# lonelycorn/mvSLAM

Measured on AMD Instinct MI355X. Metric: image-pairs/sec (2k kp, 50k RANSAC hyp), higher is better.
Workload: dtype f64; 1 GPU; 512 independent synthetic 640x480 pairs per GPU, 2000 keypoints (256-bit descriptors), 50000 8-point hypotheses per pair, full match+RANSAC+decompose+triangulate; pairs_per_gpu=512, keypoints=2000, hypotheses=50000, parallelism=pairs sharded, dp1, streams=2

## Files before the change

mvslam_amd/csrc/capi.hip:

```cpp
#include <dlfcn.h>
#include <hip/hip_runtime.h>

#include <algorithm>
#include <cmath>
#include <cstdio>
#include <cstdlib>
#include <cstring>
#include <functional>
#include <memory>
#include <string>
#include <type_traits>
#include <vector>

#include "kernels.hpp"

using namespace mvs;

struct HipFree {
    void operator()(void *p) const { (void)hipFree(p); }
};
using DevPtr = std::unique_ptr<void, HipFree>;
using DevBlocks = std::vector<DevPtr>;
struct DevWorkspace {
    DevPtr p;
// ... 208 lines not shown
static mvs_status ws_grow(mvs_ctx *ctx, DevWorkspace &w, size_t bytes, size_t floor = 0)
{
    if (w.bytes >= bytes)
        return MVS_OK;
    HIP_TRY(ctx, sync_stream(ctx));
    w.p.reset();
    w.bytes = 0;
    void *p = nullptr;
    HIP_TRY(ctx, hipMalloc(&p, std::max(bytes, floor)));
    w.p.reset(p);
    w.bytes = std::max(bytes, floor);
    return MVS_OK;
}

static void drop_orb_graph(mvs_ctx *ctx)
{
    if (ctx->orb_graph)
        (void)hipGraphExecDestroy(ctx->orb_graph);
    ctx->orb_graph = nullptr;
    ctx->orb_graph_valid = false;
}

struct Carve {
    size_t align, end = 0;
    size_t up(size_t x) const { return (x + align - 1) & ~(align - 1); }
    size_t take(size_t bytes)
    {
        const size_t o = up(end);
        end = o + bytes;
        return o;
    }
    size_t total() const { return up(end); }
};

static mvs_status ensure_groups(mvs_batch *b, int num_hypotheses)
{
    const int G = (num_hypotheses + kHypPerBlock - 1) / kHypPerBlock;
    if (G <= b->d.max_groups)
        return MVS_OK;
    HIP_TRY(b->ctx, sync_stream(b->ctx));
    const size_t P = (size_t)b->d.n_pairs, Hp = (size_t)G * kHypPerBlock;
    if (P * Hp >= (size_t(1) << 32))
        return MVS_ERR_CAPACITY;
    BatchDev &d = b->d;
    DevGroup g(b->ctx, b->blocks);
    g.add(d.wgbest, P * G);
    g.add(d.hyp_F, P * kHypRec * Hp);
    g.add(d.hyp_r32, P * kHypRec32 * Hp);
    g.add(d.hyp_okf, P * Hp);
    g.add(d.hyp_cnt, P * Hp);
    g.add(d.xlist, P * Hp);
    g.add(d.clist, 2 * P * Hp);
    if (!d.bound) g.add(d.bound, P);
    if (!d.box) g.add(d.box, P * 8);
    if (!d.mode) g.add(d.mode, P);
    if (!d.dense_n1) g.add(d.dense_n1, P);
    if (!d.ccount) g.add(d.ccount, P);
    if (!d.pcount) g.add(d.pcount, P);
    if (!d.cpos) g.add(d.cpos, P * kSortBins);
    if (!d.m0list) g.add(d.m0list, 2 * (P + 1));
    if (!d.xcount) g.add(d.xcount, 4);
    const mvs_status st = g.commit();
    if (st != MVS_OK)
        return st;
    d.clist2 = d.clist + P * Hp;
    d.max_groups = G;
    return MVS_OK;
}

static mvs_status alloc_refine(mvs_ctx *ctx, DevBlocks &owner, RefineDev &d, int problems, int stride, int frames,
                               const double *K)
{
    const size_t T = problems, S = stride;
    RefineDev r{};
    r.n_problems = problems;
    r.stride = stride;
    r.n_frames = frames;
    r.K = K;
    DevGroup g(ctx, owner);
    for (int f = 0; f < frames; ++f) {
        g.add(r.obs[f], T * S * 2);
        g.add(r.oinfo[f], T * S * 3);
    }
    g.add(r.pts0, T * S * 3);
    g.add(r.pinfo, T * S * 6);
    g.add(r.pts, T * S * 3);
    g.add(r.pts_tmp, T * S * 3);
    if (frames == 2)
        g.add(r.point_cov, T * S * 9);
    g.add(r.pose0, T * 12);
    g.add(r.m, T);
    g.add(r.out, T);
    const mvs_status st = g.commit();
    if (st == MVS_OK)
        d = r;
    return st;
}

#ifdef MVS_DEBUG_HOOKS
template <typename Launch>
static int probe_io(mvs_ctx *ctx, const void *const *in, const size_t *in_bytes, int n_in, void *const *outp, const size_t *out_bytes,
                    int n_out, Launch launch)
{
    HIP_TRY(ctx, hipSetDevice(ctx->device));
    unsigned char *d[8] = {};
    DevBlocks tmp;
    DevGroup g(ctx, tmp);
// ... 657 lines not shown
    return MVS_OK;
}

mvs_status mvs_batch_upload(mvs_batch *b, int first, int count, const uint8_t *base_desc, const float *base_kp,
                            const int32_t *n_base, const uint8_t *pair_desc, const float *pair_kp,
                            const int32_t *n_pair, const double *K, const int64_t *global_index)
{
    return batch_upload_impl(b, first, count, base_desc, base_kp, n_base, pair_desc, pair_kp, n_pair, K, global_index, true);
}

mvs_status mvs_batch_upload_async(mvs_batch *b, int first, int count, const uint8_t *base_desc, const float *base_kp,
                                  const int32_t *n_base, const uint8_t *pair_desc, const float *pair_kp,
                                  const int32_t *n_pair, const double *K, const int64_t *global_index)
{
    return batch_upload_impl(b, first, count, base_desc, base_kp, n_base, pair_desc, pair_kp, n_pair, K, global_index, false);
}

mvs_status mvs_host_alloc(size_t bytes, void **out)
{
    if (!out || bytes == 0)
        return MVS_ERR_INVALID_ARG;
    *out = nullptr;
    return hipHostMalloc(out, bytes, hipHostMallocPortable) == hipSuccess ? MVS_OK : MVS_ERR_HIP;
}

void mvs_host_free(void *p)
{
    if (p)
        (void)hipHostFree(p);
}

static mvs_status check_params(const mvs_params *p)
{
    if (!p || p->num_hypotheses < 1 || (p->sampler != MVS_SAMPLER_IDENTITY && p->sampler != MVS_SAMPLER_PHILOX))
        return MVS_ERR_INVALID_ARG;
    return MVS_OK;
}

static BatchDev batch_view(const BatchDev &b, int first, int count, int half)
{
    BatchDev v = b;
    const size_t f = (size_t)first, N = (size_t)b.max_kp, Hp = (size_t)b.max_groups * kHypPerBlock;
    v.n_pairs = count;
    v.desc1 += f * N * b.desc_words; v.desc2 += f * N * b.desc_words;
    v.kp1 += f * N * 2; v.kp2 += f * N * 2;
    v.oct1 += f * N; v.oct2 += f * N;
    v.n1 += f; v.n2 += f;
    v.Kinv += f * 9; v.K += f * 9; v.gidx += f;
    v.knn_train += f * N; v.knn_dist += f * N;
    v.M += f; v.matches += f * N; v.pts += f * N * 4;
    v.wgbest += f * b.max_groups;
    v.hyp_F += f * Hp * kHypRec; v.hyp_r32 += f * Hp * kHypRec32;
    v.hyp_okf += f * Hp; v.hyp_cnt += f * Hp;
    v.bound += f; v.box += f * 8; v.mode += f;
    v.clist += f * Hp; v.clist2 += f * Hp; v.cpos += f * kSortBins;
    v.ccount += f; v.pcount += f; v.dense_n1 += f;
    v.m0list += (size_t)half * ((size_t)b.n_pairs + 1);
    v.xlist += f * Hp;
    v.xcount += 2 * half;
    v.cand_pts += f * 4 * N * 3; v.fin += f; v.inl += f * N; v.okf += f * 4 * N;
    v.results += f; v.mask += f * N; v.points += f * N * 3; v.point_idx += f * N;
    return v;
}

constexpr int kHalvesMinPairs = 64;

static void enqueue_stages(const BatchDev &d, const RunParams &rp, int n_active, bool stats, hipStream_t s, hipEvent_t *ev,
                           LaunchTimer *lt, bool with_match = true)
{
    if (ev) (void)hipEventRecord(ev[0], s);
    if (with_match)
        launch_match_topk(d, rp, n_active, s, lt);
    if (ev) (void)hipEventRecord(ev[1], s);
    if (with_match)
        launch_match_compact(d, rp, n_active, s, lt);
    if (ev) (void)hipEventRecord(ev[2], s);
    launch_ransac(d, rp, n_active, stats, s, lt);
    if (ev) (void)hipEventRecord(ev[3], s);
    launch_finalize(d, rp, n_active, kFinalizeFull, s, lt);
    if (ev) (void)hipEventRecord(ev[4], s);
}

static mvs_status enqueue_pipeline(mvs_batch *b, const RunParams &rp, int n_active, bool stats, hipEvent_t *ev,
                                   LaunchTimer *lt = nullptr, bool with_match = true)
{
    mvs_ctx *ctx = b->ctx;
    hipStream_t s = ctx->stream;
    const bool halves = n_active >= kHalvesMinPairs && !stats && !ev && !lt && !b->d.hyp_count && ctx->half_batches;
    if (!halves) {
        enqueue_stages(b->d, rp, n_active, stats, s, ev, lt, with_match);
    } else {
        const int na = (n_active + 1) / 2;
        HIP_TRY(ctx, hipEventRecord(ctx->ev_fork, s));
        HIP_TRY(ctx, hipStreamWaitEvent(ctx->side, ctx->ev_fork, 0));
        enqueue_stages(batch_view(b->d, 0, na, 0), rp, na, false, s, nullptr, nullptr, with_match);
        const hipError_t e_first = hipGetLastError();
        enqueue_stages(batch_view(b->d, na, n_active - na, 1), rp, n_active - na, false, ctx->side, nullptr, nullptr, with_match);
        const hipError_t e_second = hipGetLastError();
        hipError_t e_join = hipEventRecord(ctx->ev_join, ctx->side);
        if (e_join == hipSuccess)
            e_join = hipStreamWaitEvent(s, ctx->ev_join, 0);
        if (e_join != hipSuccess)
            (void)hipStreamSynchronize(ctx->side);
        HIP_TRY(ctx, e_first);
        HIP_TRY(ctx, e_second);
        HIP_TRY(ctx, e_join);
    }
// ... 2196 lines not shown
```

mvslam_amd/csrc/device_math.hpp:

```cpp
#pragma once
#include <hip/hip_runtime.h>
#include <stdint.h>

#define MVS_DEV __device__ __forceinline__

namespace mvs {

constexpr double kEps = 2.220446049250313e-16;
constexpr double kTol = kEps * 1000.0;
constexpr double kJacobiEps = kEps * 10.0;
constexpr double kMinVal = 2.2250738585072014e-308;
constexpr double kSqrt2 = 1.4142135623730951;

MVS_DEV double dfma(double a, double b, double c) { return __builtin_fma(a, b, c); }
MVS_DEV double dsqrt(double a) { return __builtin_sqrt(a); }
MVS_DEV double dabs(double a) { return __builtin_fabs(a); }

MVS_DEV void rotate_inplace(double &x, double &y, double c, double s)
{
    double t0, t1;
    asm("v_mul_f64 %0, %4, %3\n\t"
        "v_mul_f64 %1, %4, %2\n\t"
        "v_fma_f64 %3, %5, %3, -%1\n\t"
        "v_fma_f64 %2, %5, %2, %0"
// ... 317 lines not shown
        double sd = W[i];
        for (int ii = 0; ii < 100 && sd <= kMinVal; ++ii) {
            const double val0 = 1.0 / 3.0;
#pragma unroll
            for (int k = 0; k < 3; ++k)
                At[i][k] = (cvrng_next(rng) & 256u) != 0 ? val0 : -val0;
#pragma unroll
            for (int it = 0; it < 2; ++it) {
#pragma unroll
                for (int j = 0; j < 3; ++j) {
                    if (j < i) {
                        sd = 0.0;
#pragma unroll
                        for (int k = 0; k < 3; ++k)
                            sd += At[i][k] * At[j][k];
                        double asum = 0.0;
#pragma unroll
                        for (int k = 0; k < 3; ++k) {
                            const double t = At[i][k] - sd * At[j][k];
                            At[i][k] = t;
                            asum += dabs(t);
                        }
                        asum = asum > kJacobiEps * 100.0 ? 1.0 / asum : 0.0;
#pragma unroll
                        for (int k = 0; k < 3; ++k)
                            At[i][k] *= asum;
                    }
                }
            }
            sd = 0.0;
#pragma unroll
            for (int k = 0; k < 3; ++k)
                sd += At[i][k] * At[i][k];
            sd = dsqrt(sd);
        }
        const double s = sd > kMinVal ? 1.0 / sd : 0.0;
#pragma unroll
        for (int k = 0; k < 3; ++k)
            At[i][k] *= s;
    }
#pragma unroll
    for (int i = 0; i < 3; ++i)
#pragma unroll
        for (int j = 0; j < 3; ++j)
            U[i][j] = At[j][i];
}
MVS_DEV void svd3_full(const double (&A)[3][3], double (&w)[3], double (&U)[3][3], double (&Vt)[3][3], unsigned &rot,
                       unsigned &pairs)
{
    bool bad3 = false;
    svd3_full<false, false, false>(A, w, U, Vt, rot, pairs, bad3);
}

MVS_DEV void philox4x32_10(uint32_t c0, uint32_t c1, uint32_t c2, uint32_t c3, uint32_t k0, uint32_t k1,
                           uint32_t (&out)[4])
{
#pragma unroll
    for (int r = 0; r < 10; ++r) {
        const uint64_t p0 = (uint64_t)0xD2511F53u * c0, p1 = (uint64_t)0xCD9E8D57u * c2;
        const uint32_t hi0 = (uint32_t)(p0 >> 32), lo0 = (uint32_t)p0;
        const uint32_t hi1 = (uint32_t)(p1 >> 32), lo1 = (uint32_t)p1;
        const uint32_t n0 = hi1 ^ c1 ^ k0, n2 = hi0 ^ c3 ^ k1;
        c0 = n0; c1 = lo1; c2 = n2; c3 = lo0;
        k0 += 0x9E3779B9u;
        k1 += 0xBB67AE85u;
    }
    out[0] = c0; out[1] = c1; out[2] = c2; out[3] = c3;
}

MVS_DEV void sample8(uint64_t seed, uint32_t hyp, int M, int sampler, int (&idx)[8])
{
    if (sampler == 0) {
#pragma unroll
        for (int k = 0; k < 8; ++k)
            idx[k] = k;
        return;
    }
    uint32_t w[8];
    {
        uint32_t o[4];
        philox4x32_10(hyp, 0u, 0u, 0u, (uint32_t)seed, (uint32_t)(seed >> 32), o);
        w[0] = o[0]; w[1] = o[1]; w[2] = o[2]; w[3] = o[3];
        philox4x32_10(hyp, 1u, 0u, 0u, (uint32_t)seed, (uint32_t)(seed >> 32), o);
        w[4] = o[0]; w[5] = o[1]; w[6] = o[2]; w[7] = o[3];
    }
    int sorted[8];
#pragma unroll
    for (int k = 0; k < 8; ++k)
        sorted[k] = 0x7fffffff;
#pragma unroll
    for (int k = 0; k < 8; ++k) {
        uint32_t r = __umulhi(w[k], (uint32_t)(M - k));
#pragma unroll
        for (int t = 0; t < 8; ++t)
            if (t < k && r >= (uint32_t)sorted[t])
                ++r;
        idx[k] = (int)r;
        int carry = (int)r;
#pragma unroll
        for (int t = 0; t < 8; ++t) {
            if (t <= k) {
                const int cur = sorted[t];
                const bool sw = carry < cur;
                sorted[t] = sw ? carry : cur;
                carry = sw ? cur : carry;
            }
        }
    }
}

MVS_DEV bool normalise8(const double (&px)[8], const double (&py)[8], double (&nx)[8], double (&ny)[8], double &scale,
                        double &mx, double &my)
{
    mx = 0.0;
    my = 0.0;
#pragma unroll
    for (int i = 0; i < 8; ++i) {
        mx += px[i];
        my += py[i];
    }
    mx *= 0.125;
    my *= 0.125;
    double sc = 0.0;
#pragma unroll
    for (int i = 0; i < 8; ++i) {
        const double dx = px[i] - mx, dy = py[i] - my;
        nx[i] = dx;
        ny[i] = dy;
        sc += dsqrt(dx * dx + dy * dy);
    }
    sc *= 0.125;
    const bool ok = sc > kEps;
    sc = kSqrt2 / sc;
#pragma unroll
    for (int i = 0; i < 8; ++i) {
        nx[i] *= sc;
        ny[i] *= sc;
    }
    scale = sc;
    return ok;
}

struct EightNorm {
    double s1, s2, m1x, m1y, m2x, m2y;
};

MVS_DEV bool eight_point_front(const double (&x1)[8], const double (&y1)[8], const double (&x2)[8], const double (&y2)[8],
                               double (&At)[9][9], EightNorm &nm)
{
    double a1[8], b1[8], a2[8], b2[8];
    bool ok = normalise8(x1, y1, a1, b1, nm.s1, nm.m1x, nm.m1y);
    ok = normalise8(x2, y2, a2, b2, nm.s2, nm.m2x, nm.m2y) && ok;
    double A[8][9];
#pragma unroll
    for (int i = 0; i < 8; ++i) {
        A[i][0] = a2[i] * a1[i]; A[i][1] = a2[i] * b1[i]; A[i][2] = a2[i];
        A[i][3] = b2[i] * a1[i]; A[i][4] = b2[i] * b1[i]; A[i][5] = b2[i];
        A[i][6] = a1[i];         A[i][7] = b1[i];         A[i][8] = 1.0;
    }
#pragma unroll
    for (int i = 0; i < 9; ++i) {
#pragma unroll
// ... 109 lines not shown
```

mvslam_amd/csrc/kernels.hip:

```cpp
#include <algorithm>
#include "kernels.hpp"

#include "device_math.hpp"
#include "prescreen.hpp"

namespace mvs {

constexpr uint32_t kKeyNone = 0xffffffffu;
__device__ __forceinline__ uint32_t bcnt_acc(uint32_t x, uint32_t acc)
{
    uint32_t r;
    asm("v_bcnt_u32_b32 %0, %1, %2" : "=v"(r) : "v"(x), "v"(acc));
    return r;
}
__device__ __forceinline__ void key_insert(uint32_t &k0, uint32_t &k1, uint32_t k)
{
    uint32_t m;
    asm("v_med3_u32 %0, %1, %2, %3" : "=v"(m) : "v"(k0), "v"(k1), "v"(k));
    k1 = m;
    k0 = min(k0, k);
}

constexpr int kTopkWaves = 16;
constexpr int kTopkTileBytes = 65536;
// ... 538 lines not shown
    for (int k = 0; k < 9; ++k)
        Fo[k] = F[k];
    Fo[9] = pair_max_error_sq(b, rp, pair);
    b.hyp_okf[(size_t)pair * Hp + h] = ok ? kPsExact : kPsInvalid;
    if (h == 0)
        b.bound[pair] = 0;
}


__global__ __launch_bounds__(256) void mode0_list_kernel(BatchDev b, int n_active)
{
    __shared__ int s_cnt[4];
    __shared__ int s_total;
    const int tid = threadIdx.x, lane = tid & 63, w = tid >> 6;
    if (tid == 0)
        s_total = 0;
    __syncthreads();
    for (int p0 = 0; p0 < n_active; p0 += 256) {
        const int pair = p0 + tid;
        const bool take = pair < n_active && b.M[pair] >= 8 && b.mode[pair] == 0;
        const unsigned long long m = __ballot(take);
        if (lane == 0)
            s_cnt[w] = __popcll(m);
        __syncthreads();
        int base = s_total;
        for (int k = 0; k < w; ++k)
            base += s_cnt[k];
        if (take)
            b.m0list[1 + base + __popcll(m & ((1ull << lane) - 1ull))] = pair;
        __syncthreads();
        if (tid == 0)
            s_total += s_cnt[0] + s_cnt[1] + s_cnt[2] + s_cnt[3];
        __syncthreads();
    }
    if (tid == 0)
        b.m0list[0] = s_total;
}

__global__ __launch_bounds__(256, 1) void ransac_solve_list_kernel(BatchDev b, RunParams rp, int blocks_per_pair)
{
    const int n_items = b.m0list[0] * blocks_per_pair;
    for (int item = blockIdx.x; item < n_items; item += gridDim.x) {
        const int pair = b.m0list[1 + item / blocks_per_pair];
        solve_record(b, rp, pair, b.M[pair], (uint32_t)(item % blocks_per_pair) * 64u + threadIdx.x);
    }
}

constexpr int kCntSlots = 4;
typedef __attribute__((address_space(4))) double CDouble;


__device__ __forceinline__ PairBox load_box(const BatchDev &b, int pair)
{
    const double *q = b.box + (size_t)pair * 8;
    PairBox bx;
    bx.x1lo = q[0]; bx.x1hi = q[1]; bx.y1lo = q[2]; bx.y1hi = q[3];
    bx.x2lo = q[4]; bx.x2hi = q[5]; bx.y2lo = q[6]; bx.y2hi = q[7];
    return bx;
}

__device__ __forceinline__ int prescreen_sample(uint64_t seed, uint32_t hyp, int M, int sampler, const double *P, double *park,
                                                const PairBox &bx, double thr, double (&F)[9], double &band, double &e32,
                                                bool &bad3)
{
    int idx[8];
    sample8(seed, hyp, M, sampler, idx);
    return prescreen_hypothesis(P, idx, park, bx, thr, F, band, e32, bad3);
}

__global__ __launch_bounds__(256) void pair_prepare_kernel(BatchDev b, RunParams rp, int force_mode)
{
    __shared__ double s_red[4][8];
    __shared__ double s_park[kPsParked * 64];
    const int pair = blockIdx.x, tid = threadIdx.x, lane = tid & 63, w = tid >> 6;
    const int M = min(b.M[pair], b.max_kp);
    if (pair == 0 && tid < 2)
        b.xcount[tid] = 0u;
    if (tid == 0) {
        b.bound[pair] = 0;
        b.ccount[pair] = 0;
        b.pcount[pair] = 0;
    }
    if (M < 8) {
        if (tid == 0)
            b.mode[pair] = 0;
        return;
    }
    const double4 *P4 = reinterpret_cast<const double4 *>(b.pts + (size_t)pair * b.max_kp * 4);
    const double big = 0x1p1000;
    double lo[4] = {big, big, big, big}, hi[4] = {-big, -big, -big, -big};
    for (int i = tid; i < M; i += 256) {
        const double4 p = P4[i];
        const double v[4] = {p.x, p.y, p.z, p.w};
#pragma unroll
        for (int k = 0; k < 4; ++k) {
            lo[k] = fmin(lo[k], v[k]);
            hi[k] = fmax(hi[k], v[k]);
        }
    }
#pragma unroll
    for (int k = 0; k < 4; ++k) {
#pragma unroll
        for (int o = 32; o > 0; o >>= 1) {
            lo[k] = fmin(lo[k], __shfl_xor(lo[k], o));
            hi[k] = fmax(hi[k], __shfl_xor(hi[k], o));
        }
    }
    if (lane == 0) {
#pragma unroll
        for (int k = 0; k < 4; ++k) {
            s_red[w][2 * k] = lo[k];
            s_red[w][2 * k + 1] = hi[k];
        }
    }
    __syncthreads();
    PairBox bx;
    {
        double q[8];
#pragma unroll
        for (int k = 0; k < 8; ++k) {
            const double a0 = s_red[0][k], a1 = s_red[1][k], a2 = s_red[2][k], a3 = s_red[3][k];
            q[k] = (k & 1) ? fmax(fmax(a0, a1), fmax(a2, a3)) : fmin(fmin(a0, a1), fmin(a2, a3));
        }
        bx.x1lo = q[0]; bx.x1hi = q[1]; bx.y1lo = q[2]; bx.y1hi = q[3];
        bx.x2lo = q[4]; bx.x2hi = q[5]; bx.y2lo = q[6]; bx.y2hi = q[7];
        if (tid < 8)
            b.box[(size_t)pair * 8 + tid] = q[tid];
    }
    if (w == 0) {
        const int H = rp.num_hypotheses;
        const uint64_t seed = rp.seed + (uint64_t)b.gidx[pair];
        const double thr = pair_max_error_sq(b, rp, pair);
        const uint32_t hh = (uint32_t)min(lane, H - 1);
        double F[9], band, e32;
        bool bad3 = false;
        int flag = prescreen_sample(seed, hh, M, rp.sampler, reinterpret_cast<const double *>(P4), s_park + lane, bx, thr, F, band, e32,
                                    bad3);
        if (bad3 && flag == kPsApprox)
            flag = kPsNeedExact;
        const bool live = lane < H;
        const int n_ok = __popcll(__ballot(live && flag != kPsInvalid));
        const int n_s64 = __popcll(__ballot(live && flag == kPsApprox && band <= kPsProbeFrac * thr));
        const int n_s32 = __popcll(__ballot(live && flag == kPsApprox && band + e32 <= kPsProbeFrac * thr &&
                                            band + 65.0 * e32 <= kPsProbeMfmaFrac * thr));
        const int mode = n_ok == 0 ? 0 : 3 * n_s32 >= n_ok ? 1 : 3 * n_s64 >= n_ok ? 2 : 0;
        if (lane == 0)
            b.mode[pair] = force_mode >= 0 ? force_mode : mode;
    }
}

__global__ __launch_bounds__(64) __attribute__((amdgpu_waves_per_eu(3, 3))) void ransac_prescreen_kernel(BatchDev b, RunParams rp)
{
    __shared__ double s_park[kPsParked * 64];
    const int pair = blockIdx.y, lane = threadIdx.x;
    const int M = b.M[pair];
    if (M < 8 || b.mode[pair] == 0)
        return;
    const int H = rp.num_hypotheses;
    const uint32_t h = blockIdx.x * 64 + lane;
    const bool live = h < (uint32_t)H;
    const uint32_t hh = live ? h : (uint32_t)(H - 1);
    const uint64_t seed = rp.seed + (uint64_t)b.gidx[pair];
    const double *P = b.pts + (size_t)pair * b.max_kp * 4;
    const PairBox bx = load_box(b, pair);
    const double thr = pair_max_error_sq(b, rp, pair);
    double F[9], band, e32;
    bool bad3 = false;
    int flag = prescreen_sample(seed, hh, M, rp.sampler, P, s_park + lane, bx, thr, F, band, e32, bad3);
    const int mode = b.mode[pair];
    const double btot = mode == 1 ? band + e32 : band;
    if (flag == kPsApprox && (bad3 || !(btot <= kPsBandFrac * thr)))
        flag = kPsNeedExact;
    if (!live)
        flag = kPsInvalid;
    const size_t Hp = (size_t)b.max_groups * kHypPerBlock;
    const size_t rec = (size_t)pair * Hp + h;
    double *Fo = b.hyp_F + rec * kHypRec;
    if (mode == 1) {
        float *fo = b.hyp_r32 + rec * kHypRec32;
        float q[12];
// ... 1112 lines not shown
                        F[k] = f[k];
                    c = 0;
#pragma unroll 4
                    for (int i = 0; i < M; ++i) {
                        const double4 p = L4[i];
                        c += epipolar_residual(F, p.x, p.y, p.z, p.w) < thr ? 1 : 0;
                    }
                }
                s_cnt[q] = c;
            }
        } else if (b.mode[pair] != 0) {
            for (int q = w; q < n_list; q += kSelThreads / 64) {
                if (okb[s_list[q]] == kPsInvalid) {
                    if (lane == 0)
                        s_cnt[q] = -1;
                    continue;
                }
                const double *f = Fp + (size_t)s_list[q] * kHypRec;
                double F[9];
#pragma unroll
                for (int k = 0; k < 9; ++k)
                    F[k] = f[k];
                int c = 0;
                for (int i = lane; i < M; i += 64) {
                    const double4 p = P4[i];
                    c += epipolar_residual(F, p.x, p.y, p.z, p.w) < thr ? 1 : 0;
                }
#pragma unroll
                for (int o = 32; o > 0; o >>= 1)
                    c += __shfl_xor(c, o);
                if (lane == 0)
                    s_cnt[q] = c;
            }
        } else {
            for (int q = tid; q < n_list; q += kSelThreads)
                s_cnt[q] = cntp[s_list[q]];
        }
        __syncthreads();
        {
            int cm = -1;
            for (int q = tid; q < n_list; q += kSelThreads)
                cm = max(cm, s_cnt[q]);
#pragma unroll
            for (int o = 32; o > 0; o >>= 1)
                cm = max(cm, __shfl_xor(cm, o));
            if (lane == 0)
                s_tot[w] = cm;
            __syncthreads();
            const int target = max(max(max(s_tot[0], s_tot[1]), max(s_tot[2], s_tot[3])), s_best.cnt);
            __syncthreads();
            int n_ties = 0;
            for (int q0 = 0; q0 < n_list; q0 += kSelThreads) {
                const int q = q0 + tid;
                const bool tie = q < n_list && s_cnt[q] == target;
                const uint32_t hq = q < n_list ? s_list[q] : 0u;
                const unsigned long long bal = __ballot(tie);
                if (lane == 0)
                    s_tot[w] = __popcll(bal);
                __syncthreads();
                int off = n_ties, tot = 0;
#pragma unroll
                for (int k = 0; k < 4; ++k) {
                    const int v = s_tot[k];
                    off += (k < w) ? v : 0;
                    tot += v;
                }
                if (tie)
                    s_list[off + __popcll(bal & ((1ull << lane) - 1ull))] = hq;
                n_ties += tot;
                __syncthreads();
            }
            n_list = n_ties;
        }
        if (n_list == 0)
            continue;
        if (n_list <= kSelSerial) {
            staged = false;
            for (int q = 0; q < n_list; ++q) {
                const uint32_t h = s_list[q];
                if (tid < 9)
                    s_F[tid] = Fp[(size_t)h * kHypRec + tid];
                __syncthreads();
                double F[9];
#pragma unroll
                for (int k = 0; k < 9; ++k)
                    F[k] = s_F[k];
                int n_in = 0;
                for (int start = 0; start < M; start += kSelThreads) {
                    const int i = start + tid;
                    double r = 0.0;
                    bool in = false;
                    if (i < M) {
                        const double4 p = P4[i];
                        r = epipolar_residual(F, p.x, p.y, p.z, p.w);
                        in = r < thr;
                    }
                    const unsigned long long bal = __ballot(in);
                    if (lane == 0)
                        s_tot[w] = __popcll(bal);
                    __syncthreads();
                    int off = n_in, tot = 0;
#pragma unroll
                    for (int k = 0; k < 4; ++k) {
                        const int v = s_tot[k];
                        off += (k < w) ? v : 0;
                        tot += v;
                    }
// ... 1010 lines not shown
```

mvslam_amd/csrc/kernels.hpp:

```cpp
#pragma once
#include <hip/hip_runtime.h>
#include <stdint.h>

#include "../../include/mvslam_hip.h"

namespace mvs {

constexpr int kMaxKp = 4096;
constexpr int kSortBins = kMaxKp + 1;
constexpr int kHypPerBlock = 256;
constexpr int kMaxDescWords = 16;
constexpr int kHypRec = 10;
constexpr int kHypRec32 = 12;

struct WgBest {
    int32_t count;
    uint32_t hyp;
    double residual;
    double F[9];
};
static_assert(sizeof(WgBest) == 88, "WgBest layout");

struct FinModel {
    double R[2][9];
    double Rr[2][9];
    double T[3];
    int32_t n_inl;
    int32_t ncand;
    int32_t proceed;
    int32_t npre;
    int32_t pre_cnt[4];
    int32_t best_c;
    int32_t pad[3];
};

struct BatchDev {
    int n_pairs;
    int max_kp;
    int desc_words;
    int max_groups;
    int cu_count;

    const uint32_t *desc1;
    const uint32_t *desc2;
    const float *kp1;
    const float *kp2;
    const uint8_t *oct1;
    const uint8_t *oct2;
    const int32_t *n1;
    const int32_t *n2;
    const double *Kinv;
    const double *K;
    const int64_t *gidx;

    int32_t *knn_train;
    int32_t *knn_dist;
    int32_t *M;
    mvs_match *matches;
    double *pts;
    WgBest *wgbest;
// ... 342 lines not shown
```

mvslam_amd/csrc/prescreen.hpp:

```cpp
#pragma once
#include "device_math.hpp"

namespace mvs {

struct PairBox {
    double x1lo, x1hi, y1lo, y1hi, x2lo, x2hi, y2lo, y2hi;
};

constexpr double kPsU = 0x1p-53;
constexpr double kPsTauC = 2.0e-12;
constexpr double kPsEtaQ = 4.0e-12;
constexpr double kPsSvd3 = 2.0e-11;
constexpr double kPsTrip = 1.0e-12;
constexpr double kPsBandFrac = 4.0;
constexpr double kPsProbeFrac = 0.125;
constexpr double kPsProbeMfmaFrac = 1.25;
constexpr int kPsInvalid = 0, kPsApprox = 1, kPsNeedExact = 2, kPsExact = 3;

MVS_DEV double recip_guarded(double x) { return div_fast(1.0, x); }

MVS_DEV double sqrt_bound(double x)
{
    const double y = __builtin_amdgcn_rsq(x);
    double g = x * y;
    const double h = y * 0.5;
    const double r = dfma(-h, g, 0.5);
    g = dfma(g, r, g);
    const double d = dfma(-g, g, x);
    return dfma(d, h, g);
}
MVS_DEV double sqrt_bound0(double x)
{
    const double g = sqrt_bound(x);
    return x < 0x1p-700 ? 0.0 : g;
}
MVS_DEV double rcp_bound(double x)
{
    double r = __builtin_amdgcn_rcp(x);
    double e = dfma(-x, r, 1.0);
    r = dfma(r, e, r);
    e = dfma(-x, r, 1.0);
    return dfma(r, e, r);
}

MVS_DEV bool sample_norm(const double (&px)[8], const double (&py)[8], double &scale, double &mx, double &my, bool &tiny)
{
    mx = 0.0;
    my = 0.0;
#pragma unroll
    for (int i = 0; i < 8; ++i) {
        mx += px[i];
        my += py[i];
    }
    mx *= 0.125;
    my *= 0.125;
    double sc = 0.0;
#pragma unroll
    for (int i = 0; i < 8; ++i) {
        const double dx = px[i] - mx, dy = py[i] - my;
        const double q = dx * dx + dy * dy;
        tiny = tiny | ((q != 0.0) & !sqrt_fast_ok(q));
        sc += sqrt_fast(q);
    }
    sc *= 0.125;
    const bool ok = sc > kEps;
    scale = kSqrt2 / sc;
    return ok;
}

MVS_DEV void prescreen_rank2(const double (&g)[9], double (&X)[9], double &e_out, double &sige_out, double &extra_out,
                             double &s2lb_out, bool &ok_out)
{
    const double c00 = dfma(g[6], g[6], dfma(g[3], g[3], g[0] * g[0]));
    const double c01 = dfma(g[6], g[7], dfma(g[3], g[4], g[0] * g[1]));
    const double c02 = dfma(g[6], g[8], dfma(g[3], g[5], g[0] * g[2]));
    const double c11 = dfma(g[7], g[7], dfma(g[4], g[4], g[1] * g[1]));
    const double c12 = dfma(g[7], g[8], dfma(g[4], g[5], g[1] * g[2]));
    const double c22 = dfma(g[8], g[8], dfma(g[5], g[5], g[2] * g[2]));
    const double k2 = (c00 + c11) + c22;
    const double k1 = dfma(c00, c11, -(c01 * c01)) + dfma(c00, c22, -(c02 * c02)) + dfma(c11, c22, -(c12 * c12));
    const double dg = dfma(g[0], dfma(g[4], g[8], -(g[5] * g[7])),
                           dfma(-g[1], dfma(g[3], g[8], -(g[5] * g[6])), g[2] * dfma(g[3], g[7], -(g[4] * g[6]))));
    const double k0 = dg * dg;
    const double m2k2 = -2.0 * k2;
    double lam = 0.0;
#pragma unroll
    for (int it = 0; it < 8; ++it) {
        const double f = dfma(dfma(lam - k2, lam, k1), lam, -k0);
        const double fp = dfma(dfma(3.0, lam, m2k2), lam, k1);
        double r = __builtin_amdgcn_rcp(fp);
        r = r * dfma(-fp, r, 2.0);
        lam = dfma(-f, r, lam);
    }
    const double m00 = c00 - lam, m11 = c11 - lam, m22 = c22 - lam;
    const double ax = dfma(c01, c12, -(c02 * m11)), ay = dfma(c02, c01, -(m00 * c12)), az = dfma(m00, m11, -(c01 * c01));
    const double bx = dfma(c01, m22, -(c02 * c12)), by = dfma(c02, c02, -(m00 * m22)), bz = dfma(m00, c12, -(c01 * c02));
    const double cx = dfma(m11, m22, -(c12 * c12)), cy = dfma(c12, c02, -(c01 * m22)), cz = dfma(c01, c12, -(m11 * c02));
    const double na = dfma(az, az, dfma(ay, ay, ax * ax));
    const double nb = dfma(bz, bz, dfma(by, by, bx * bx));
    const double nc = dfma(cz, cz, dfma(cy, cy, cx * cx));
    const bool ub = nb > na;
    double vx = ub ? bx : ax, vy = ub ? by : ay, vz = ub ? bz : az, nv = ub ? nb : na;
    const bool uc = nc > nv;
    vx = uc ? cx : vx; vy = uc ? cy : vy; vz = uc ? cz : vz; nv = uc ? nc : nv;
    bool ok = nv >= 0x1p-190;
    double h;
    (void)sqrt_fast_nz_h(nv, h);
    h += h;
    vx *= h; vy *= h; vz *= h;
    const double w0 = dfma(g[2], vz, dfma(g[1], vy, g[0] * vx));
    const double w1 = dfma(g[5], vz, dfma(g[4], vy, g[3] * vx));
    const double w2 = dfma(g[8], vz, dfma(g[7], vy, g[6] * vx));
    X[0] = dfma(-w0, vx, g[0]); X[1] = dfma(-w0, vy, g[1]); X[2] = dfma(-w0, vz, g[2]);
    X[3] = dfma(-w1, vx, g[3]); X[4] = dfma(-w1, vy, g[4]); X[5] = dfma(-w1, vz, g[5]);
    X[6] = dfma(-w2, vx, g[6]); X[7] = dfma(-w2, vy, g[7]); X[8] = dfma(-w2, vz, g[8]);
    const double sg2 = dfma(w2, w2, dfma(w1, w1, w0 * w0));
    const double sig = dsqrt(sg2);
    const double rs = div_fast(1.0, fmax(sig, 0x1p-190));
    const double u0 = w0 * rs, u1 = w1 * rs, u2 = w2 * rs;
    const double e0 = dfma(g[6], u2, dfma(g[3], u1, dfma(g[0], u0, -(sig * vx))));
// ... 1 lines not shown
    const double e2 = dfma(g[8], u2, dfma(g[5], u1, dfma(g[2], u0, -(sig * vz))));
    const double eps2 = sqrt_bound0(dfma(e2, e2, dfma(e1, e1, e0 * e0))) * (1.0 + 1e-14);
    const bool useA = (eps2 < sig) && (sig >= 0x1p-190);
    e_out = (useA ? eps2 : sig) + kPsTrip;
    sige_out = useA ? sig : 0.0;
    extra_out = useA ? eps2 + kPsTrip : kPsTrip;
    ok = ok && (sig == sig);
    const double q1 = dfma(X[8], X[8], dfma(X[7], X[7], dfma(X[6], X[6], dfma(X[5], X[5], dfma(X[4], X[4],
                      dfma(X[3], X[3], dfma(X[2], X[2], dfma(X[1], X[1], X[0] * X[0]))))))));
    const double t00 = dfma(X[6], X[6], dfma(X[3], X[3], X[0] * X[0]));
    const double t01 = dfma(X[6], X[7], dfma(X[3], X[4], X[0] * X[1]));
    const double t02 = dfma(X[6], X[8], dfma(X[3], X[5], X[0] * X[2]));
    const double t11 = dfma(X[7], X[7], dfma(X[4], X[4], X[1] * X[1]));
    const double t12 = dfma(X[7], X[8], dfma(X[4], X[5], X[1] * X[2]));
    const double t22 = dfma(X[8], X[8], dfma(X[5], X[5], X[2] * X[2]));
    const double off = dfma(t12, t12, dfma(t02, t02, t01 * t01));
    const double q2 = dfma(2.0, off, dfma(t22, t22, dfma(t11, t11, t00 * t00)));
    const double q1q = q1 * q1;
    const double Pm = 0.5 * (q1q - q2) - 4e-15;
    const double disc = fmax(dfma(-4.0, Pm, q1q), 0.0) + 1e-13;
    const double s2q = (Pm + Pm) / (q1 * (1.0 + 1e-13) + dsqrt(disc));
    s2lb_out = s2q > 0.0 ? dsqrt(s2q) * (1.0 - 1e-14) : 0.0;
    ok_out = ok && (q1 <= 1.5);
}

MVS_DEV void prescreen_denormalise(const double (&Fn)[9], const EightNorm &nm, double (&F)[9])
{
    const double s1 = nm.s1, s2 = nm.s2;
    const double tx1 = -nm.m1x * s1, ty1 = -nm.m1y * s1, tx2 = -nm.m2x * s2, ty2 = -nm.m2y * s2;
    double G[3][3];
#pragma unroll
    for (int j = 0; j < 3; ++j) {
        G[0][j] = s2 * Fn[j];
        G[1][j] = s2 * Fn[3 + j];
        G[2][j] = dfma(tx2, Fn[j], dfma(ty2, Fn[3 + j], Fn[6 + j]));
    }
#pragma unroll
    for (int i = 0; i < 3; ++i) {
        F[i * 3 + 0] = G[i][0] * s1;
        F[i * 3 + 1] = G[i][1] * s1;
        F[i * 3 + 2] = dfma(G[i][0], tx1, dfma(G[i][1], ty1, G[i][2]));
    }
}

constexpr int kPsTri = 28;
constexpr int kPsParked = 26;
MVS_DEV constexpr int ps_tri(int i, int k) { return k * (k - 1) / 2 + i; }

MVS_DEV int prescreen_hypothesis(const double *P, int (&idx)[8], double *park, const PairBox &bx, double thr, double (&F)[9],
                                 double &band_out, double &e32_out, bool &bad3)
{
    EightNorm nm;
    bool ok, tiny = false;
    {
        double x1[8], y1[8], x2[8], y2[8];
#pragma unroll
        for (int k = 0; k < 8; ++k) {
            const double4 p = *reinterpret_cast<const double4 *>(P + (size_t)idx[k] * 4);
            x1[k] = p.x; y1[k] = p.y; x2[k] = p.z; y2[k] = p.w;
        }
        ok = sample_norm(x1, y1, nm.s1, nm.m1x, nm.m1y, tiny);
        ok = sample_norm(x2, y2, nm.s2, nm.m2x, nm.m2y, tiny) && ok;
    }
    band_out = 0.0;
    e32_out = 0.0;
    if (!ok && !tiny) {
#pragma unroll
        for (int k = 0; k < 9; ++k)
            F[k] = 0.0;
        return kPsInvalid;
    }
    double v[8][9];
    double rlast[kPsTri - kPsParked];
    double rd[8], beta[8];
    double S = 0.0;
    bool piv_ok = !tiny;
#pragma unroll
    for (int j = 0; j < 8; ++j) {
        double col[9];
        {
            if (j < 2)
                asm volatile("" : "+v"(idx[j]));
            else
                asm volatile("" : "+v"(idx[j]) : "v"(beta[j > 1 ? j - 2 : 0]));
            const double4 p = *reinterpret_cast<const double4 *>(P + (size_t)idx[j] * 4);
            const double a1 = (p.x - nm.m1x) * nm.s1, b1 = (p.y - nm.m1y) * nm.s1;
            const double a2 = (p.z - nm.m2x) * nm.s2, b2 = (p.w - nm.m2y) * nm.s2;
            col[0] = a2 * a1; col[1] = a2 * b1; col[2] = a2;
            col[3] = b2 * a1; col[4] = b2 * b1; col[5] = b2;
            col[6] = a1;      col[7] = b1;      col[8] = 1.0;
            S = dfma(dfma(a2, a2, dfma(b2, b2, 1.0)), dfma(a1, a1, dfma(b1, b1, 1.0)), S);
        }
#pragma unroll
        for (int k = 0; k < j; ++k) {
            double d = 0.0, d1 = 0.0;
#pragma unroll
            for (int i = k; i < 9; i += 2) {
                d = dfma(v[k][i], col[i], d);
                if (i + 1 < 9)
                    d1 = dfma(v[k][i + 1], col[i + 1], d1);
            }
            d += d1;
            const double t = beta[k] * d;
#pragma unroll
            for (int i = k; i < 9; ++i)
                col[i] = dfma(-t, v[k][i], col[i]);
            if (ps_tri(k, j) < kPsParked)
                park[ps_tri(k, j) * 64] = col[k];
            else
                rlast[ps_tri(k, j) - kPsParked] = col[k];
        }
        double ss = 0.0;
#pragma unroll
        for (int i = j; i < 9; ++i)
            ss = dfma(col[i], col[i], ss);
        piv_ok = piv_ok && (ss >= 0x1p-190);
        double hn;
        const double nrm = sqrt_fast_nz_h(ss, hn);
        const double x0 = col[j];
        const double alpha = x0 >= 0.0 ? -nrm : nrm;
        const double vv = nrm * (nrm + dabs(x0));
        double iv = hn + hn;
        iv = dfma(iv, dfma(-nrm, iv, 1.0), iv);
        rd[j] = x0 >= 0.0 ? -iv : iv;
        beta[j] = rcp_bound(vv);
        v[j][j] = x0 - alpha;
#pragma unroll
        for (int i = j + 1; i < 9; ++i)
            v[j][i] = col[i];
    }
    S *= 1.0 + 1e-12;
    piv_ok = piv_ok && (S <= 0x1p100);
    const double sqrtS = sqrt_bound(S) * (1.0 + 1e-12);
    double n[9];
#pragma unroll
    for (int i = 0; i < 9; ++i)
        n[i] = i == 8 ? 1.0 : 0.0;
#pragma unroll
// ... 6 lines not shown
                d1 = dfma(v[k][i + 1], n[i + 1], d1);
        }
        d += d1;
        const double t = beta[k] * d;
#pragma unroll
        for (int i = k; i < 9; ++i)
            n[i] = dfma(-t, v[k][i], n[i]);
    }
    double y2sum = 0.0;
    {
        double R[kPsTri];
#pragma unroll
        for (int q = 0; q < kPsTri; ++q)
            R[q] = q < kPsParked ? park[q * 64] : rlast[q - kPsParked];
        double inv[8];
#pragma unroll
        for (int i = 0; i < 8; ++i)
            inv[i] = rd[i];
#pragma unroll
        for (int j = 0; j < 8; ++j) {
            double y[8];
            y[j] = inv[j];
            y2sum = dfma(y[j], y[j], y2sum);
#pragma unroll
            for (int i = j - 1; i >= 0; --i) {
                double s = 0.0;
#pragma unroll
                for (int k = i + 1; k <= j; ++k)
                    s = dfma(R[ps_tri(i, k)], y[k], s);
                y[i] = -(s * inv[i]);
                y2sum = dfma(y[i], y[i], y2sum);
            }
        }
    }
    const double yf = sqrt_bound(y2sum) * (1.0 + 1e-12);
    const double rho = 1.8e-13 * sqrtS;
    const double z = 16.0 * kPsU * sqrtS * yf;
    const double sig8 = (1.0 - z) * rcp_bound(yf) * (1.0 - 1e-13) - 4e-14 * sqrtS;
    const double rg = rcp_bound(sig8);
    const double eta_j = 1.01 * kPsTauC * S * (rg * rg) + kPsEtaQ;
    const double eta_a = 1.5 * rho * rg + 1e-13;
    double Fn[9], e3, sige, extra, s2lb;
    bool ok3;
    prescreen_rank2(n, Fn, e3, sige, extra, s2lb, ok3);
    prescreen_denormalise(Fn, nm, F);
    bad3 = false;
    const double eta = (eta_j + eta_a + e3 + kPsSvd3) * (1.0 + 1e-12);
    const double delta = ((s2lb - extra) - sige) - eta;
    const double dfn = (2.0 + 2.0 * (sige + 3.0 * eta) * rcp_bound(delta) * (1.0 + 1e-14)) * eta + extra + kPsSvd3;
    const double d1x = fmax(dabs(nm.m1x - bx.x1lo), dabs(nm.m1x - bx.x1hi));
    const double d1y = fmax(dabs(nm.m1y - bx.y1lo), dabs(nm.m1y - bx.y1hi));
    const double d2x = fmax(dabs(nm.m2x - bx.x2lo), dabs(nm.m2x - bx.x2hi));
    const double d2y = fmax(dabs(nm.m2y - bx.y2lo), dabs(nm.m2y - bx.y2hi));
    const double e1x = fmax(dabs(bx.x1lo), dabs(bx.x1hi)) + dabs(nm.m1x);
    const double e1y = fmax(dabs(bx.y1lo), dabs(bx.y1hi)) + dabs(nm.m1y);
    const double e2x = fmax(dabs(bx.x2lo), dabs(bx.x2hi)) + dabs(nm.m2x);
    const double e2y = fmax(dabs(bx.y2lo), dabs(bx.y2hi)) + dabs(nm.m2y);
    const double s1q = nm.s1 * nm.s1, s2q = nm.s2 * nm.s2;
    const double n12 = dfma(s1q, dfma(d1x, d1x, d1y * d1y), 1.0) * dfma(s2q, dfma(d2x, d2x, d2y * d2y), 1.0);
    const double n12p = dfma(s1q, dfma(e1x, e1x, e1y * e1y), 1.0) * dfma(s2q, dfma(e2x, e2x, e2y * e2y), 1.0);
    const double band = (dfn * sqrt_bound(n12) * (1.0 + 1e-9) + 64.0 * kPsU * sqrt_bound(n12p)) * (1.0 + 1e-9) + 1e-15 * thr;
    band_out = band;
    {
        const double X1 = fmax(dabs(bx.x1lo), dabs(bx.x1hi)), Y1 = fmax(dabs(bx.y1lo), dabs(bx.y1hi));
        const double X2 = fmax(dabs(bx.x2lo), dabs(bx.x2hi)), Y2 = fmax(dabs(bx.y2lo), dabs(bx.y2hi));
        const double t0 = dfma(X2, dabs(F[0]), dfma(Y2, dabs(F[3]), dabs(F[6])));
        const double t1 = dfma(X2, dabs(F[1]), dfma(Y2, dabs(F[4]), dabs(F[7])));
        const double t2 = dfma(X2, dabs(F[2]), dfma(Y2, dabs(F[5]), dabs(F[8])));
        const double T = dfma(t0, X1, dfma(t1, Y1, t2));
        e32_out = 16.0 * 0x1p-24 * T * (1.0 + 1e-6) + 1e-30;
    }
    const bool certified = piv_ok && ok3 && (z < 0.5) && (sig8 > 0.0) && (delta > 0.0) && (eta < 1e-3) && (band < 0x1p100);
    return certified ? kPsApprox : kPsNeedExact;
}

}
```

Before: 115,900 pairs/s.

## Precompute box abs-max, fast sample normalisation, and med3-based sorted sampler

Stores per-pair absolute-max box extents once in the box record (widened to 12 doubles) so the prescreen no longer recomputes them per hypothesis. Replaces the exact sample normalisation with a fast nonzero sqrt path, falling back to the exact version only when a wave sees tiny or non-finite values. Rewrites the 8-index sampler's insertion sort using min/max/median-of-three and byte offsets for point loads. It also adds a guard so tie detection ignores negative targets. The intent is to cut per-hypothesis ALU work in the RANSAC hypothesis kernel, at the cost of a larger box record and a divergent fallback branch.

```diff
diff --git a/mvslam_amd/csrc/capi.hip b/mvslam_amd/csrc/capi.hip
--- a/mvslam_amd/csrc/capi.hip
+++ b/mvslam_amd/csrc/capi.hip
@@ -284,7 +284,7 @@
     g.add(d.xlist, P * Hp);
     g.add(d.clist, 2 * P * Hp);
     if (!d.bound) g.add(d.bound, P);
-    if (!d.box) g.add(d.box, P * 8);
+    if (!d.box) g.add(d.box, P * kBoxRec);
     if (!d.mode) g.add(d.mode, P);
     if (!d.dense_n1) g.add(d.dense_n1, P);
     if (!d.ccount) g.add(d.ccount, P);
@@ -1048,7 +1048,7 @@
     v.wgbest += f * b.max_groups;
     v.hyp_F += f * Hp * kHypRec; v.hyp_r32 += f * Hp * kHypRec32;
     v.hyp_okf += f * Hp; v.hyp_cnt += f * Hp;
-    v.bound += f; v.box += f * 8; v.mode += f;
+    v.bound += f; v.box += f * kBoxRec; v.mode += f;
     v.clist += f * Hp; v.clist2 += f * Hp; v.cpos += f * kSortBins;
     v.ccount += f; v.pcount += f; v.dense_n1 += f;
     v.m0list += (size_t)half * ((size_t)b.n_pairs + 1);
diff --git a/mvslam_amd/csrc/device_math.hpp b/mvslam_amd/csrc/device_math.hpp
--- a/mvslam_amd/csrc/device_math.hpp
+++ b/mvslam_amd/csrc/device_math.hpp
@@ -393,62 +393,9 @@
     svd3_full<false, false, false>(A, w, U, Vt, rot, pairs, bad3);
 }
 
-MVS_DEV void philox4x32_10(uint32_t c0, uint32_t c1, uint32_t c2, uint32_t c3, uint32_t k0, uint32_t k1,
-                           uint32_t (&out)[4])
-{
-#pragma unroll
-    for (int r = 0; r < 10; ++r) {
-        const uint64_t p0 = (uint64_t)0xD2511F53u * c0, p1 = (uint64_t)0xCD9E8D57u * c2;
-        const uint32_t hi0 = (uint32_t)(p0 >> 32), lo0 = (uint32_t)p0;
-        const uint32_t hi1 = (uint32_t)(p1 >> 32), lo1 = (uint32_t)p1;
-        const uint32_t n0 = hi1 ^ c1 ^ k0, n2 = hi0 ^ c3 ^ k1;
-        c0 = n0; c1 = lo1; c2 = n2; c3 = lo0;
-        k0 += 0x9E3779B9u;
-        k1 += 0xBB67AE85u;
-    }
-    out[0] = c0; out[1] = c1; out[2] = c2; out[3] = c3;
-}
-
-MVS_DEV void sample8(uint64_t seed, uint32_t hyp, int M, int sampler, int (&idx)[8])
-{
-    if (sampler == 0) {
-#pragma unroll
-        for (int k = 0; k < 8; ++k)
-            idx[k] = k;
-        return;
-    }
-    uint32_t w[8];
-    {
-        uint32_t o[4];
-        philox4x32_10(hyp, 0u, 0u, 0u, (uint32_t)seed, (uint32_t)(seed >> 32), o);
-        w[0] = o[0]; w[1] = o[1]; w[2] = o[2]; w[3] = o[3];
-        philox4x32_10(hyp, 1u, 0u, 0u, (uint32_t)seed, (uint32_t)(seed >> 32), o);
-        w[4] = o[0]; w[5] = o[1]; w[6] = o[2]; w[7] = o[3];
-    }
-    int sorted[8];
-#pragma unroll
-    for (int k = 0; k < 8; ++k)
-        sorted[k] = 0x7fffffff;
-#pragma unroll
-    for (int k = 0; k < 8; ++k) {
-        uint32_t r = __umulhi(w[k], (uint32_t)(M - k));
-#pragma unroll
-        for (int t = 0; t < 8; ++t)
-            if (t < k && r >= (uint32_t)sorted[t])
-                ++r;
-        idx[k] = (int)r;
-        int carry = (int)r;
-#pragma unroll
-        for (int t = 0; t < 8; ++t) {
-            if (t <= k) {
-                const int cur = sorted[t];
-                const bool sw = carry < cur;
-                sorted[t] = sw ? carry : cur;
-                carry = sw ? cur : carry;
-            }
-        }
-    }
-}
+}
+#include "sampler.hpp"
+namespace mvs {
 
 MVS_DEV bool normalise8(const double (&px)[8], const double (&py)[8], double (&nx)[8], double (&ny)[8], double &scale,
                         double &mx, double &my)
diff --git a/mvslam_amd/csrc/kernels.hip b/mvslam_amd/csrc/kernels.hip
--- a/mvslam_amd/csrc/kernels.hip
+++ b/mvslam_amd/csrc/kernels.hip
@@ -614,10 +614,11 @@
 
 __device__ __forceinline__ PairBox load_box(const BatchDev &b, int pair)
 {
-    const double *q = b.box + (size_t)pair * 8;
+    const double *q = b.box + (size_t)pair * kBoxRec;
     PairBox bx;
     bx.x1lo = q[0]; bx.x1hi = q[1]; bx.y1lo = q[2]; bx.y1hi = q[3];
     bx.x2lo = q[4]; bx.x2hi = q[5]; bx.y2lo = q[6]; bx.y2hi = q[7];
+    bx.ax1 = q[8]; bx.ay1 = q[9]; bx.ax2 = q[10]; bx.ay2 = q[11];
     return bx;
 }
 
@@ -686,8 +687,12 @@
         }
         bx.x1lo = q[0]; bx.x1hi = q[1]; bx.y1lo = q[2]; bx.y1hi = q[3];
         bx.x2lo = q[4]; bx.x2hi = q[5]; bx.y2lo = q[6]; bx.y2hi = q[7];
+        box_abs_max(bx);
+        const double a[4] = {bx.ax1, bx.ay1, bx.ax2, bx.ay2};
         if (tid < 8)
-            b.box[(size_t)pair * 8 + tid] = q[tid];
+            b.box[(size_t)pair * kBoxRec + tid] = q[tid];
+        else if (tid < kBoxRec)
+            b.box[(size_t)pair * kBoxRec + tid] = tid == 8 ? a[0] : tid == 9 ? a[1] : tid == 10 ? a[2] : a[3];
     }
     if (w == 0) {
         const int H = rp.num_hypotheses;
@@ -1906,7 +1911,7 @@
             int n_ties = 0;
             for (int q0 = 0; q0 < n_list; q0 += kSelThreads) {
                 const int q = q0 + tid;
-                const bool tie = q < n_list && s_cnt[q] == target;
+                const bool tie = q < n_list && target >= 0 && s_cnt[q] == target;
                 const uint32_t hq = q < n_list ? s_list[q] : 0u;
                 const unsigned long long bal = __ballot(tie);
                 if (lane == 0)
diff --git a/mvslam_amd/csrc/kernels.hpp b/mvslam_amd/csrc/kernels.hpp
--- a/mvslam_amd/csrc/kernels.hpp
+++ b/mvslam_amd/csrc/kernels.hpp
@@ -6,6 +6,7 @@
 
 namespace mvs {
 
+constexpr int kBoxRec = 12;
 constexpr int kMaxKp = 4096;
 constexpr int kSortBins = kMaxKp + 1;
 constexpr int kHypPerBlock = 256;
diff --git a/mvslam_amd/csrc/prescreen.hpp b/mvslam_amd/csrc/prescreen.hpp
--- a/mvslam_amd/csrc/prescreen.hpp
+++ b/mvslam_amd/csrc/prescreen.hpp
@@ -5,7 +5,15 @@
 
 struct PairBox {
     double x1lo, x1hi, y1lo, y1hi, x2lo, x2hi, y2lo, y2hi;
+    double ax1, ay1, ax2, ay2;
 };
+MVS_DEV void box_abs_max(PairBox &bx)
+{
+    bx.ax1 = fmax(dabs(bx.x1lo), dabs(bx.x1hi));
+    bx.ay1 = fmax(dabs(bx.y1lo), dabs(bx.y1hi));
+    bx.ax2 = fmax(dabs(bx.x2lo), dabs(bx.x2hi));
+    bx.ay2 = fmax(dabs(bx.y2lo), dabs(bx.y2hi));
+}
 
 constexpr double kPsU = 0x1p-53;
 constexpr double kPsTauC = 2.0e-12;
@@ -66,6 +74,31 @@
     const bool ok = sc > kEps;
     scale = kSqrt2 / sc;
     return ok;
+}
+
+MVS_DEV double sample_norm_nz(const double (&px)[8], const double (&py)[8], double &scale, double &mx, double &my, double &qmin)
+{
+    mx = 0.0;
+    my = 0.0;
+#pragma unroll
+    for (int i = 0; i < 8; ++i) {
+        mx += px[i];
+        my += py[i];
+    }
+    mx *= 0.125;
+    my *= 0.125;
+    double sc = 0.0;
+#pragma unroll
+    for (int i = 0; i < 8; ++i) {
+        const double dx = px[i] - mx, dy = py[i] - my;
+        const double q = dx * dx + dy * dy;
+        qmin = fmin(qmin, q);
+        double h;
+        sc += sqrt_fast_nz_h(q, h);
+    }
+    sc *= 0.125;
+    scale = kSqrt2 / sc;
+    return sc;
 }
 
 MVS_DEV void prescreen_rank2(const double (&g)[9], double (&X)[9], double &e_out, double &sige_out, double &extra_out,
@@ -173,15 +206,27 @@
 {
     EightNorm nm;
     bool ok, tiny = false;
+    uint32_t off[8];
+#pragma unroll
+    for (int k = 0; k < 8; ++k)
+        off[k] = (uint32_t)idx[k] << 5;
+    const char *Pb = reinterpret_cast<const char *>(P);
     {
         double x1[8], y1[8], x2[8], y2[8];
 #pragma unroll
         for (int k = 0; k < 8; ++k) {
-            const double4 p = *reinterpret_cast<const double4 *>(P + (size_t)idx[k] * 4);
+            const double4 p = *reinterpret_cast<const double4 *>(Pb + off[k]);
             x1[k] = p.x; y1[k] = p.y; x2[k] = p.z; y2[k] = p.w;
         }
-        ok = sample_norm(x1, y1, nm.s1, nm.m1x, nm.m1y, tiny);
-        ok = sample_norm(x2, y2, nm.s2, nm.m2x, nm.m2y, tiny) && ok;
+        double qmin = __builtin_inf();
+        const double sc1 = sample_norm_nz(x1, y1, nm.s1, nm.m1x, nm.m1y, qmin);
+        const double sc2 = sample_norm_nz(x2, y2, nm.s2, nm.m2x, nm.m2y, qmin);
+        ok = (sc1 > kEps) && (sc2 > kEps);
+        const bool redo = !(qmin >= 0x1p-767) || !(sc1 + sc2 < __builtin_inf());
+        if (__builtin_expect(__any(redo), 0)) {
+            ok = sample_norm(x1, y1, nm.s1, nm.m1x, nm.m1y, tiny);
+            ok = sample_norm(x2, y2, nm.s2, nm.m2x, nm.m2y, tiny) && ok;
+        }
     }
     band_out = 0.0;
     e32_out = 0.0;
@@ -201,10 +246,10 @@
         double col[9];
         {
             if (j < 2)
-                asm volatile("" : "+v"(idx[j]));
+                asm volatile("" : "+v"(off[j]));
             else
-                asm volatile("" : "+v"(idx[j]) : "v"(beta[j > 1 ? j - 2 : 0]));
-            const double4 p = *reinterpret_cast<const double4 *>(P + (size_t)idx[j] * 4);
+                asm volatile("" : "+v"(off[j]) : "v"(beta[j > 1 ? j - 2 : 0]));
+            const double4 p = *reinterpret_cast<const double4 *>(Pb + off[j]);
             const double a1 = (p.x - nm.m1x) * nm.s1, b1 = (p.y - nm.m1y) * nm.s1;
             const double a2 = (p.z - nm.m2x) * nm.s2, b2 = (p.w - nm.m2y) * nm.s2;
             col[0] = a2 * a1; col[1] = a2 * b1; col[2] = a2;
@@ -317,18 +362,17 @@
     const double d1y = fmax(dabs(nm.m1y - bx.y1lo), dabs(nm.m1y - bx.y1hi));
     const double d2x = fmax(dabs(nm.m2x - bx.x2lo), dabs(nm.m2x - bx.x2hi));
     const double d2y = fmax(dabs(nm.m2y - bx.y2lo), dabs(nm.m2y - bx.y2hi));
-    const double e1x = fmax(dabs(bx.x1lo), dabs(bx.x1hi)) + dabs(nm.m1x);
-    const double e1y = fmax(dabs(bx.y1lo), dabs(bx.y1hi)) + dabs(nm.m1y);
-    const double e2x = fmax(dabs(bx.x2lo), dabs(bx.x2hi)) + dabs(nm.m2x);
-    const double e2y = fmax(dabs(bx.y2lo), dabs(bx.y2hi)) + dabs(nm.m2y);
+    const double e1x = bx.ax1 + dabs(nm.m1x);
+    const double e1y = bx.ay1 + dabs(nm.m1y);
+    const double e2x = bx.ax2 + dabs(nm.m2x);
+    const double e2y = bx.ay2 + dabs(nm.m2y);
     const double s1q = nm.s1 * nm.s1, s2q = nm.s2 * nm.s2;
     const double n12 = dfma(s1q, dfma(d1x, d1x, d1y * d1y), 1.0) * dfma(s2q, dfma(d2x, d2x, d2y * d2y), 1.0);
     const double n12p = dfma(s1q, dfma(e1x, e1x, e1y * e1y), 1.0) * dfma(s2q, dfma(e2x, e2x, e2y * e2y), 1.0);
     const double band = (dfn * sqrt_bound(n12) * (1.0 + 1e-9) + 64.0 * kPsU * sqrt_bound(n12p)) * (1.0 + 1e-9) + 1e-15 * thr;
     band_out = band;
     {
-        const double X1 = fmax(dabs(bx.x1lo), dabs(bx.x1hi)), Y1 = fmax(dabs(bx.y1lo), dabs(bx.y1hi));
-        const double X2 = fmax(dabs(bx.x2lo), dabs(bx.x2hi)), Y2 = fmax(dabs(bx.y2lo), dabs(bx.y2hi));
+        const double X1 = bx.ax1, Y1 = bx.ay1, X2 = bx.ax2, Y2 = bx.ay2;
         const double t0 = dfma(X2, dabs(F[0]), dfma(Y2, dabs(F[3]), dabs(F[6])));
         const double t1 = dfma(X2, dabs(F[1]), dfma(Y2, dabs(F[4]), dabs(F[7])));
         const double t2 = dfma(X2, dabs(F[2]), dfma(Y2, dabs(F[5]), dabs(F[8])));
diff --git a/mvslam_amd/csrc/sampler.hpp b/mvslam_amd/csrc/sampler.hpp
--- /dev/null
+++ b/mvslam_amd/csrc/sampler.hpp
@@ -0,0 +1,65 @@
+#pragma once
+#include <stdint.h>
+#ifndef MVS_DEV
+#include <hip/hip_runtime.h>
+#define MVS_DEV __device__ __forceinline__
+#endif
+
+namespace mvs {
+
+MVS_DEV void philox4x32_10(uint32_t c0, uint32_t c1, uint32_t c2, uint32_t c3, uint32_t k0, uint32_t k1,
+                           uint32_t (&out)[4])
+{
+#pragma unroll
+    for (int r = 0; r < 10; ++r) {
+        const uint64_t p0 = (uint64_t)0xD2511F53u * c0, p1 = (uint64_t)0xCD9E8D57u * c2;
+        const uint32_t hi0 = (uint32_t)(p0 >> 32), lo0 = (uint32_t)p0;
+        const uint32_t hi1 = (uint32_t)(p1 >> 32), lo1 = (uint32_t)p1;
+        const uint32_t n0 = hi1 ^ c1 ^ k0, n2 = hi0 ^ c3 ^ k1;
+        c0 = n0; c1 = lo1; c2 = n2; c3 = lo0;
+        k0 += 0x9E3779B9u;
+        k1 += 0xBB67AE85u;
+    }
+    out[0] = c0; out[1] = c1; out[2] = c2; out[3] = c3;
+}
+
+MVS_DEV uint32_t umin32(uint32_t a, uint32_t b) { return a < b ? a : b; }
+MVS_DEV uint32_t umax32(uint32_t a, uint32_t b) { return a > b ? a : b; }
+MVS_DEV uint32_t umed3(uint32_t a, uint32_t b, uint32_t c) { return umax32(umin32(a, b), umin32(umax32(a, b), c)); }
+
+MVS_DEV void sample8(uint64_t seed, uint32_t hyp, int M, int sampler, int (&idx)[8])
+{
+    if (sampler == 0) {
+#pragma unroll
+        for (int k = 0; k < 8; ++k)
+            idx[k] = k;
+        return;
+    }
+    uint32_t w[8];
+    {
+        uint32_t o[4];
+        philox4x32_10(hyp, 0u, 0u, 0u, (uint32_t)seed, (uint32_t)(seed >> 32), o);
+        w[0] = o[0]; w[1] = o[1]; w[2] = o[2]; w[3] = o[3];
+        philox4x32_10(hyp, 1u, 0u, 0u, (uint32_t)seed, (uint32_t)(seed >> 32), o);
+        w[4] = o[0]; w[5] = o[1]; w[6] = o[2]; w[7] = o[3];
+    }
+    uint32_t sorted[8];
+#pragma unroll
+    for (int k = 0; k < 8; ++k) {
+        uint32_t r = __umulhi(w[k], (uint32_t)(M - k));
+#pragma unroll
+        for (int t = 0; t < k; ++t)
+            r += r >= sorted[t] ? 1u : 0u;
+        idx[k] = (int)r;
+        if (k < 7) {
+            if (k > 0)
+                sorted[k] = umax32(sorted[k - 1], r);
+#pragma unroll
+            for (int t = k - 1; t > 0; --t)
+                sorted[t] = umed3(sorted[t - 1], sorted[t], r);
+            sorted[0] = k > 0 ? umin32(sorted[0], r) : r;
+        }
+    }
+}
+
+}
```

After: 117,700 pairs/s (median of 6 runs). Within noise of the previous version (+1.5%).
